# MilchRatchet/Luminary

Hardware: AMD Instinct MI355X
Metric: Mrays/s at 1920x1080, 8 bounces (higher is better)
Workload: dtype f32

## Files before the change

### luminary_amd/csrc/device/dev_scene.h

```cpp
#pragma once

#include <hip/hip_vector_types.h>
#include <stdint.h>

namespace lum {

struct alignas(128) Bvh4Node {
  float lo_x[4], lo_y[4], lo_z[4];
  float hi_x[4], hi_y[4], hi_z[4];
  uint32_t child[4];
  uint32_t pad[4];
};
static_assert(sizeof(Bvh4Node) == 128, "BVH4 node must be one cache line");

#ifndef LUM_BVH8
#define LUM_BVH8 0
#endif
struct alignas(128) Bvh8Node {
  float origin[3];
  uint8_t exp[3], pad0;
  uint32_t child[8];
  uint8_t lo_x[8], lo_y[8], lo_z[8], hi_x[8], hi_y[8], hi_z[8];
  uint32_t pad[8];
};
// ... 127 lines not shown
#endif
  const uint2* sobol_table;
  uint32_t sobol_first, sobol_count, sobol_stride;
};

struct PathQueue {
  float4* origin_t;
  float4* dir_slot;
  uint4* aux;
  uint4* hit_id;
  uint32_t* hit_scene_tri;
  uint32_t* parent;
};
constexpr uint32_t kParentDeferred = 0x80000000u, kParentMask = 0x7FFFFFFFu;

struct NeeQueue {
  float4* geo_color_light;
  float4* bsdf_ray_prob;
  float4* bsdf_weight_sum;
  uint4* ambient;
  uint4* sun;
  uint32_t* amb_path;
  float4* sun_water;
  float4* amb_t1;
  float4* amb_t2;
};

struct ShadowQueue {
  float4* origin_dist;
  float4* dir_out;
  uint4* ids;
  float4* vis;
  uint32_t* light_items;
  uint32_t capacity;
};

struct FusedResolve {
  PathQueue prev;
  NeeQueue nee_prev;
  ShadowQueue fallback;
  uint32_t* ended;
  const uint32_t* ended_prev;
};

constexpr uint32_t kVolumeShadowKinds = 19, kVolumeKindSun = 15, kVolumeKindAmbient = 16, kVolumeKindSun2 = 17, kVolumeKindAmbient2 = 18;
constexpr uint32_t kShadowKindAmbient2 = 4, kShadowKindSun2 = 5, kSurfaceShadowKindsWater = 6;
struct CloudQueue {
  uint32_t* items;
  float4* result;
  float* hit_dist;
  uint32_t capacity;
};
struct VolumeQueue {
  float4* bridge;
  uint4* sky;
  float4* weight;
  float4* sun_water;
  float4* amb_t1;
  float4* amb_t2;
  uint32_t* items;
};

struct PassParams {
  const uint32_t* pixels;
  uint32_t num_pixels, batch, first_sample;
};
// ... 58 lines not shown
```

### luminary_amd/csrc/device/kernels.h

```cpp
#pragma once

#include "kernel_shadow.h"
#include "dev_sky.h"
#include "dev_volume.h"
#include "dev_particle.h"
#include "dev_water.h"
#include "dev_cloud_march.h"

LUM_NS_BEGIN

constexpr int kBlock = 256;
#ifndef LUM_SHADE_WAVES
#define LUM_SHADE_WAVES 3
#endif
#ifndef LUM_CLOUD_WAVES
#define LUM_CLOUD_WAVES 4
#endif
#ifndef LUM_CLOUD_PERSISTENT
#define LUM_CLOUD_PERSISTENT 1
#endif
#ifndef LUM_HIT_COMPACT
#define LUM_HIT_COMPACT 1
#endif
#ifndef LUM_FEATURE_WAVES
// ... 167 lines not shown
  if (mat.roughness_tex != kTextureNone) roughness = texture_load(sc, mat.roughness_tex, tex_coords, true, make_float4(0.5f, 0.0f, 0.0f, 0.0f)).x;
  if (mat.flags & kDMatRoughnessAsSmoothness) roughness = 1.0f - roughness;
  roughness = fmaxf(roughness, 2e-2f);
  if ((state & kStDeltaPath) == 0) roughness = fmaxf(roughness, mat.roughness_clamp);
  uint32_t flags = mat.flags & kDMatSubstrateMask;
  if (mat.metallic_tex == kTextureNone && (mat.flags & kDMatMetallic)) flags |= kMatMetallic;
  if (mat.flags & kDMatColoredTransparency) flags |= kMatColoredTransparency;
  if (inside) flags |= kMatRefractionInside;
  const float other_ior = medium_ior_peek(medium, inside);
  const float ior_in = inside ? mat.refraction_index : other_ior;
  const float ior_out = inside ? other_ior : mat.refraction_index;
  if (((flags & kMatSubstrateMask) == kMatTranslucent) && (fabsf(1.0f - ior_in / ior_out) < 1e-4f)) {
    if ((flags & kMatColoredTransparency) == 0) albedo = col(lerpf(1.0f, albedo.r, alpha), lerpf(1.0f, albedo.g, alpha), lerpf(1.0f, albedo.b, alpha));
    alpha = 0.0f;
    flags |= kMatColoredTransparency;
  }
  GeoContext g;
  g.instance_id = inst; g.tri_id = tri;
  g.normal = xf_rot(tf, normal);
  g.face_normal_packed = normal_pack(face);
  g.position = position;
  g.V = ray_world * -1.0f;
  g.state = state;
  g.params.flags = flags;
  g.params.set(albedo, alpha, roughness, emission, ior_in / ior_out);
  return g;
}

LUM_DEV void add_to_result(float4* results, uint32_t slot, Col v) {
  if (!any_positive(v)) return;
  float4 r = results[slot];
  r.x += v.r; r.y += v.g; r.z += v.b;
  results[slot] = r;
}

struct ResolveRecords { uint4 aux; uint32_t slot; float4 cl, lc; uint4 amb; };
LUM_DEV ResolveRecords load_resolve_records(const PathQueue& in, const NeeQueue& nee, uint32_t i) {
  ResolveRecords r;
  r.aux = ld_stream(&in.aux[i]);
  r.slot = fbits(reinterpret_cast<const float*>(&in.dir_slot[i])[3]);
  r.cl = ld_stream(&nee.geo_color_light[i]);
  r.lc = ld_stream(&nee.bsdf_weight_sum[i]);
  r.amb = ld_stream(&nee.ambient[i]);
  return r;
}
template <int kAmbient>
LUM_DEV bool resolve_records(const DeviceScene& sc, const PathQueue& in, const NeeQueue& nee, const ShadowQueue& sq, float4* results, uint32_t i, bool lights_present, float ambient_vis,
                             const ResolveRecords& r, const uint32_t* hit_word = nullptr) {
  const uint4 aux = r.aux;
  const uint32_t slot = r.slot;
  const bool geo_allowed = lights_present && ((aux.w & kStVolumeScattered) == 0);
  const float4 cl = r.cl, lc = r.lc;
  const uint4 amb = r.amb;
  const bool deferred = kAmbient == 2 && hit_word != nullptr;
  const bool need_geo = fbits(cl.w) != kLightIdInvalid && geo_allowed, need_bsdf = lc.w != 0.0f, need_amb = kAmbient != 1 && !deferred && (amb.x != 0 || amb.y != 0);
  const float4 zero = make_float4(0.0f, 0.0f, 0.0f, 0.0f);
  float4 vg = zero, vb = zero, va = zero;
  uint32_t word = 0u;
  if (deferred) word = *hit_word;
  if (need_geo) vg = ld_stream(&sq.vis[i]);
  if (need_bsdf) vb = ld_stream(&sq.vis[sq.capacity + i]);
  if (need_amb) va = ld_stream(&sq.vis[2u * sq.capacity + i]);
  const float4 before = results[slot];
  if (deferred) {
    if (!(word & kHitTriHit)) { if (word & kHitTriCutout) return false; ambient_vis = 1.0f; }
    else { if ((word & (kHitTriBeyondEps | kHitTriOpaque)) != (kHitTriBeyondEps | kHitTriOpaque)) return false; ambient_vis = 0.0f; }
// ... 361 lines not shown
        LUM_LAP(clock, 4);
        if (kSkyMode != kSkyConstantColor) {
          uint4 sun = make_uint4(0u, 0u, 0u, 0u);
          Col sun_light; V3 sun_dir;
          bool have_sun;
          if (kWater && top_volume == kVolumeOcean) have_sun = sun_caustic_sample(sc, sky_view(sc), g, smp, 0u, top_volume, second_volume, sun_light, sun_dir);
          else {
            have_sun = sample_sun(sc, sky_view(sc), lf, g, smp, sun_light, sun_dir);
            if (have_sun && top_volume != kVolumeNone) sun_light = sun_light * volume_transmittance(sc, top_volume, g.position, sun_dir, kFltMax);
          }
          if (have_sun) {
            const U2 c = record_pack(sun_light), r = ray_pack(sun_dir);
            sun = make_uint4(c.x, c.y, r.x, r.y);
            if (c.x != 0 || c.y != 0) {
              want_sun = true;
              const V3 ar = ray_unpack(r);
              s_sun_dir = make_float4(ar.x, ar.y, ar.z, kFltMax);
              if (kWater) {
                const SkyRayPlan plan = plan_sun_ray(sc, hit_origin, hid.x, top_volume, true, ar);
                s_sun_dir.w = plan.limit;
                nee.sun_water[i] = make_float4(plan.fresnel_factor, 0.0f, 0.0f, bitsf(sky_ray_flags(plan)));
                if (plan.second && !plan.total_reflection) {
                  want_sun2 = true;
                  s_sun2_o = make_float4(plan.second_origin.x, plan.second_origin.y, plan.second_origin.z, kFltMax);
                  s_sun2_d = make_float4(plan.second_dir.x, plan.second_dir.y, plan.second_dir.z, 0.0f);
                }
              }
            }
          }
          st_stream(&nee.sun[i], sun);
          LUM_LAP(clock, 5);
        }
        if (kStage == 0) st_stream(&nee.geo_color_light[i], geo_cl);
        st_stream(&nee.bsdf_ray_prob[i], bs_rp); st_stream(&nee.bsdf_weight_sum[i], bs_ws);
        st_stream(&nee.ambient[i], amb);

        const float roughness = g.params.roughness();
        bool is_delta;
        if (bounce.transparent_pass) {
          const float ior = g.params.ior();
          const float rs = (ior >= 1.0f) ? ior : 1.0f / ior;
          is_delta = roughness * fminf(rs - 1.0f, 1.0f) <= 0.05f;
        }
        else is_delta = bounce.microfacet_based && (roughness <= 0.05f);
        const bool pass_through = is_pass_through(g, bounce);

        Col record = record_in;
        const Col emission = g.params.emission();
        if (any_positive(emission)) add_to_result(results, slot, emission * record);
        record = record * bounce.weight;

        uint32_t new_state = state | kStUseIgnoreHandle;
        if (kSkyMode != kSkyDefault && !pass_through) new_state &= ~kStAllowAmbient; else new_state |= kStAllowAmbient;
        if (!is_delta) new_state &= ~kStDeltaPath;
        if (!pass_through) new_state &= ~(kStCameraDirection | kStAllowEmission);

        survive = true;
        if ((state & kStDeltaPath) == 0) {
          const float value = importance(record);
          if (value < sc.cam_rr_threshold) {
            const float p = (value > 0.0f) ? fmaxf(value / sc.cam_rr_threshold, 1.0f / 8.0f) : 0.0f;
            if (smp.next1(kRndRussianRoulette) > p) survive = false;
            else record = record * (1.0f / p);
          }
        }
        if (survive) {
          uint32_t medium = aux.z;
// ... 1 lines not shown
            const bool inside = (g.params.flags & kMatRefractionInside) != 0;
            float new_ior = 1.0f;
            if (!inside) new_ior = medium_ior_peek(medium, inside) / g.params.ior();
            medium = medium_ior_modify(medium, new_ior, !inside);
          }
          const U2 rp = record_pack(record);
          n_o = make_float4(g.position.x, g.position.y, g.position.z, kFltMax);
          n_d = make_float4(bounce.ray.x, bounce.ray.y, bounce.ray.z, d4.w);
          n_aux = make_uint4(rp.x, rp.y, medium, new_state);
          n_hid = make_uint4(g.instance_id, g.tri_id, hid.z, hid.w);
        }
        }
      }
    }
    if (kStage == 1) {
      const unsigned long long bg = __ballot(want_geo);
      if (bg) {
        uint32_t base = 0;
        if (lane == (uint32_t) __builtin_ctzll(bg)) base = atomicAdd(ctrl + kCtlShadowItems, (uint32_t) __popcll(bg));
        base = __shfl(base, __builtin_ctzll(bg));
        if (want_geo) {
          const uint32_t j = base + (uint32_t) __popcll(bg & below);
          st_stream(&sq.origin_dist[j], make_float4(s_origin.x, s_origin.y, s_origin.z, s_geo_dir.w));
          st_stream(&sq.dir_out[j], make_float4(s_geo_dir.x, s_geo_dir.y, s_geo_dir.z, bitsf(i)));
          st_stream(&sq.ids[j], s_geo_ids);
        }
      }
      continue;
    }
    const bool amb_deferred = reuse_ambient && want_amb && survive;
    if (amb_deferred) { want_amb = false; vertices += 1u << 16; }
    LUM_LAP(clock, 6);
    const unsigned long long ballot = __ballot(survive);
    const unsigned long long bg = __ballot(want_geo), ba = __ballot(want_amb), bn = __ballot(want_sun), bl = __ballot(want_lq);
    const unsigned long long b2a = kWater ? __ballot(want_amb2) : 0ull, b2s = kWater ? __ballot(want_sun2) : 0ull;
    const uint32_t ng = (uint32_t) __popcll(bg), na = (uint32_t) __popcll(ba), ns = (uint32_t) __popcll(bn), na2 = (uint32_t) __popcll(b2a);
    const unsigned long long be = announce_children ? __ballot(valid && !survive) : 0ull;
    const uint32_t want_count = (lane == 0) ? (uint32_t) __popcll(ballot) : (lane == 1) ? ng + na + ns + na2 + (uint32_t) __popcll(b2s) : (lane == 2) ? (uint32_t) __popcll(bl) :
                                (lane == 3) ? (uint32_t) __popcll(be) : 0u;
    uint32_t* const want_word = (lane == 0) ? count_out : (lane == 1) ? ctrl + kCtlShadowItems : (lane == 2) ? ctrl + kCtlLightItems : ctrl + kCtlSkyItems;
    uint32_t reserved = 0;
    if (want_count) reserved = atomicAdd(want_word, want_count);
    const uint32_t base_out = __builtin_amdgcn_readlane(reserved, 0), base_shadow = __builtin_amdgcn_readlane(reserved, 1), base_light = __builtin_amdgcn_readlane(reserved, 2);
    uint32_t amb_path = kNoAmbientPath;
    if (survive) {
      const uint32_t j = base_out + (uint32_t) __popcll(ballot & below);
      st_stream(&out.origin_t[j], n_o); st_stream(&out.dir_slot[j], n_d); st_stream(&out.aux[j], n_aux); st_stream(&out.hit_id[j], n_hid);
      amb_path = amb_deferred ? j : kNoAmbientPath;
      if (announce_children) out.parent[j] = i | (amb_deferred ? kParentDeferred : 0u);
    }
    if (reuse_ambient && valid && !announce_children) nee.amb_path[i] = amb_path;
    if (be != 0ull && valid && !survive) fused_dev->ended[__builtin_amdgcn_readlane(reserved, 3) + (uint32_t) __popcll(be & below)] = i;
    if (want_geo) {
      const uint32_t j = base_shadow + (uint32_t) __popcll(bg & below);
      st_stream(&sq.origin_dist[j], make_float4(s_origin.x, s_origin.y, s_origin.z, s_geo_dir.w));
      st_stream(&sq.dir_out[j], make_float4(s_geo_dir.x, s_geo_dir.y, s_geo_dir.z, bitsf(i)));
      st_stream(&sq.ids[j], s_geo_ids);
    }
    if (want_amb) {
      const uint32_t j = base_shadow + ng + (uint32_t) __popcll(ba & below);
      st_stream(&sq.origin_dist[j], make_float4(s_origin.x, s_origin.y, s_origin.z, s_amb_dir.w));
      st_stream(&sq.dir_out[j], make_float4(s_amb_dir.x, s_amb_dir.y, s_amb_dir.z, bitsf(2u * sq.capacity + i)));
      st_stream(&sq.ids[j], make_uint4(0xFFFFFFFFu, 0u, s_geo_ids.z, s_geo_ids.w));
    }
    if (want_sun) {
      const uint32_t j = base_shadow + ng + na + (uint32_t) __popcll(bn & below);
      st_stream(&sq.origin_dist[j], make_float4(s_origin.x, s_origin.y, s_origin.z, s_sun_dir.w));
      st_stream(&sq.dir_out[j], make_float4(s_sun_dir.x, s_sun_dir.y, s_sun_dir.z, bitsf(3u * sq.capacity + i)));
      st_stream(&sq.ids[j], make_uint4(0xFFFFFFFFu, 0u, s_geo_ids.z, s_geo_ids.w));
    }
    if (kWater) {
      if (want_amb2) {
        const uint32_t j = base_shadow + ng + na + ns + (uint32_t) __popcll(b2a & below);
        sq.origin_dist[j] = s_amb2_o;
        sq.dir_out[j] = make_float4(s_amb2_d.x, s_amb2_d.y, s_amb2_d.z, bitsf(kShadowKindAmbient2 * sq.capacity + i));
        sq.ids[j] = make_uint4(0xFFFFFFFFu, 0u, 0xFFFFFFFFu, 0u);
      }
      if (want_sun2) {
        const uint32_t j = base_shadow + ng + na + ns + na2 + (uint32_t) __popcll(b2s & below);
        sq.origin_dist[j] = s_sun2_o;
        sq.dir_out[j] = make_float4(s_sun2_d.x, s_sun2_d.y, s_sun2_d.z, bitsf(kShadowKindSun2 * sq.capacity + i));
        sq.ids[j] = make_uint4(0xFFFFFFFFu, 0u, 0xFFFFFFFFu, 0u);
      }
    }
    if (want_lq) sq.light_items[base_light + (uint32_t) __popcll(bl & below)] = i;
    LUM_LAP(clock, 7);
  }
  clock.flush();
  uint32_t deferred = vertices >> 16;
  vertices &= 0xFFFFu;
#pragma unroll
  for (int off = 32; off > 0; off >>= 1) { vertices += __shfl_down(vertices, off); deferred += __shfl_down(deferred, off); }
  if ((threadIdx.x & 63) == 0 && vertices) atomicAdd((unsigned long long*) &counters[kCntVertices], (unsigned long long) vertices);
  if ((threadIdx.x & 63) == 0 && deferred) atomicAdd((unsigned long long*) &counters[kCntAmbientDeferred], (unsigned long long) deferred);
}

__global__ __launch_bounds__(kBlock) void k_shade_debug(DeviceScene sc, PathQueue in, float4* results, const uint32_t* ctrl) {
  const uint32_t n = ctrl[kCtlPaths];
  for (uint32_t i = blockIdx.x * kBlock + threadIdx.x; i < n; i += gridDim.x * kBlock) {
    const float4 o4 = in.origin_t[i], d4 = in.dir_slot[i];
    const uint4 aux = in.aux[i], hid = in.hit_id[i];
    const V3 origin = v3(o4.x, o4.y, o4.z), ray = v3(d4.x, d4.y, d4.z);
    Col result = splat(0.0f);
    if (hid.x == kHitSky) {
      if (sc.shading_mode == 1u) {
        if (sc.sky_mode == kSkyDefault) {
          if (sc.sky_lut_transmittance && sc.sky_lut_multiscattering) {
            const SkyView sky = sky_view(sc);
            const Sampler smp{sc.bluenoise_2d, hid.z & 0xFFFFu, hid.z >> 16, path_sample_id(hid.w), 0u};
            result = sky_get_color(sc, sky, world_to_sky(sky, origin), ray, kFltMax, true, (int) sky.steps, smp.next1(kRndSkyStepOffset));
          }
        }
        else if (sc.sky_mode == kSkyHdri) result = sky_hdri_color(sc, origin, ray, kStCameraDirection);
        else result = col(sc.sky_constant_color[0], sc.sky_constant_color[1], sc.sky_constant_color[2]);
      }
      else if (sc.shading_mode == 4u) result = col(0.0f, 0.63f, 1.0f);
    }
    else if (hid.x == kHitOcean) {
// ... 51 lines not shown

__global__ __launch_bounds__(kBlock, LUM_FEATURE_WAVES) void k_sky_inscattering(DeviceScene sc, PathQueue in, float4* results, const uint32_t* ctrl, uint32_t depth_const) {
  const uint32_t n = ctrl[kCtlPaths];
  const SkyView sky = sky_view(sc);
  for (uint32_t i = blockIdx.x * kBlock + threadIdx.x; i < n; i += gridDim.x * kBlock) {
    const uint4 hid = in.hit_id[i];
    if (hid.x == kHitSky) continue;
    const float4 o4 = in.origin_t[i], d4 = in.dir_slot[i];
    uint4 aux = in.aux[i];
    const Sampler smp{sc.bluenoise_2d, hid.z & 0xFFFFu, hid.z >> 16, path_sample_id(hid.w), depth_const};
    Col record = record_unpack(U2{aux.x, aux.y});
    const Col c = sky_trace_inscattering(sc, sky, world_to_sky(sky, v3(o4.x, o4.y, o4.z)), v3(d4.x, d4.y, d4.z), o4.w * 0.001f, record, depth_const == 0u,
                                         smp.next1(kRndSkyInscatteringStep), smp.next1(kRndSkyStepOffset));
    add_to_result(results, fbits(d4.w), c);
    const U2 rp = record_pack(record);
    aux.x = rp.x; aux.y = rp.y;
    in.aux[i] = aux;
  }
}

__global__ __launch_bounds__(kBlock) void k_light_query(DeviceScene sc, PathQueue in, NeeQueue nee, ShadowQueue sq, uint32_t* ctrl, uint32_t depth_const,
                                                        uint64_t* counters) {
  const uint32_t n = ctrl[kCtlLightItems];
  const uint32_t lane = threadIdx.x & 63;
  const unsigned long long below = (1ull << lane) - 1ull;
  RayStats st{0, 0, 0};
  uint32_t light_queries = 0;
  const uint32_t rounds = (n + gridDim.x * kBlock - 1) / (gridDim.x * kBlock);
  for (uint32_t round = 0; round < rounds; round++) {
    const uint32_t item = (round * gridDim.x + blockIdx.x) * kBlock + threadIdx.x;
    bool want = false;
    float4 s_origin, s_dir; uint4 s_ids; uint32_t i = 0;
    if (item < n) {
      i = sq.light_items[item];
      const uint4 hid = in.hit_id[i];
      const float4 o4 = in.origin_t[i], d4 = in.dir_slot[i];
      const V3 hit_origin = v3(o4.x, o4.y, o4.z) + v3(d4.x, d4.y, d4.z) * o4.w;
      const float4 rp = nee.bsdf_ray_prob[i], ws = nee.bsdf_weight_sum[i];
      const V3 ray = v3(rp.x, rp.y, rp.z);
      const Sampler smp{sc.bluenoise_2d, hid.z & 0xFFFFu, hid.z >> 16, path_sample_id(hid.w), depth_const};
      uint32_t num_hits = 0;
      const uint32_t light_id = light_query(sc, hit_origin, ray, hid.x, hid.y, smp.next1(kRndLightBsdfTrace), num_hits, st);
      light_queries++;
      bool valid = light_id != kLightIdInvalid;
      float dist = kFltMax;
      uint2 handle = make_uint2(0xFFFFFFFFu, 0u);
      Col lc = splat(0.0f);
      if (light_id != kLightIdInvalid) {
        handle = sc.light_tri_handles[light_id];
        const TableLight entry = load_tri_light_table(sc, light_id);
        const TriLight& tl = entry.tri;
        F2 uv;
        dist = intersect_triangle(tl.vertex, tl.edge1, tl.edge2, hit_origin, ray, uv);
        if (dist != kFltMax) {
          lc = entry.textured ? tri_light_color(sc, tl, uv) : entry.color;
          const float mis = (ws.w == 0.0f) ? 1.0f : mis_base(rp.w, tri_light_solid_angle(tl, hit_origin), importance(lc) * entry.area, dist * dist, ws.w);
          lc = lc * (mis * num_hits);
          lc = lc * col(ws.x, ws.y, ws.z);
        }
        else valid = false;
      }
      nee.bsdf_weight_sum[i] = make_float4(lc.r, lc.g, lc.b, valid ? 1.0f : 0.0f);
      if (valid && (sc.fog_active || sc.ocean_active)) {
        const Col seen = volume_transmittance(sc, sc.ocean_active ? volume_stack_peek(hid.w, false) : (uint32_t) kVolumeFog, hit_origin, ray, dist);
        nee.bsdf_ray_prob[i] = make_float4(seen.r, seen.g, seen.b, 0.0f);
      }
      if (valid) {
        want = true;
        s_origin = make_float4(hit_origin.x, hit_origin.y, hit_origin.z, dist);
        s_dir = make_float4(ray.x, ray.y, ray.z, bitsf(sq.capacity + i));
        s_ids = make_uint4(handle.x, handle.y, hid.x, hid.y);
      }
    }
    const unsigned long long bw = __ballot(want);
    if (bw) {
      uint32_t base = 0;
      if (lane == 0) base = atomicAdd(ctrl + kCtlShadowItems, (uint32_t) __popcll(bw));
      base = __builtin_amdgcn_readfirstlane(base);
      if (want) {
        const uint32_t j = base + (uint32_t) __popcll(bw & below);
        sq.origin_dist[j] = s_origin; sq.dir_out[j] = s_dir; sq.ids[j] = s_ids;
      }
    }
  }
#pragma unroll
  for (int off = 32; off > 0; off >>= 1) light_queries += __shfl_down(light_queries, off);
  if ((threadIdx.x & 63) == 0 && light_queries) atomicAdd((unsigned long long*) &counters[kCntLightBvh], (unsigned long long) light_queries);
  flush_stats(counters, st, 0, kCntLightBvh, kCntNodesLight, kCntTrisLight);
}

LUM_DEV bool resolves_here(uint32_t hit_type) {
  return !(hit_type > kHitTriangleLimit && !particle_is_hit(hit_type) && hit_type != kHitOcean);
}

__global__ __launch_bounds__(kBlock) void k_resolve(DeviceScene sc, PathQueue in, NeeQueue nee, ShadowQueue sq, float4* results, const uint32_t* ctrl) {
  const uint32_t n = ctrl[kCtlPaths];
  const bool lights_present = sc.light_tree_root != nullptr && sc.num_lights > 0;
  for (uint32_t i = blockIdx.x * kBlock + threadIdx.x; i < n; i += gridDim.x * kBlock) {
    if (!resolves_here(in.hit_id[i].x)) continue;
    resolve_vertex<false>(sc, in, nee, sq, results, i, lights_present, 0.0f);
  }
}

__global__ __launch_bounds__(kBlock) void k_resolve_ended(DeviceScene sc, PathQueue in, NeeQueue nee, ShadowQueue sq, float4* results, const uint32_t* ctrl, const uint32_t* list) {
// ... 233 lines not shown
              }
            }
          }
        }
      }
      const float random_choice = smp.next1(kRndBsdfGiResampling);
      const F2 random_dir = smp.next2(kRndBsdfGiDiffuse);
      const V3 bounce = je_phase_sample(sc.particles_phase, ray, random_dir, random_choice);
      uint4 amb = make_uint4(0u, 0u, 0u, 0u);
      if (sc.sky_mode != kSkyDefault) {
        const U2 c = record_pack(sky_color_no_compute(sc, position, bounce, 0u) * albedo), r = ray_pack(bounce);
        amb = make_uint4(c.x, c.y, r.x, r.y);
        if (c.x != 0 || c.y != 0) {
          const V3 ar = ray_unpack(r);
          if (sc.ocean_active) {
            const SkyRayPlan plan = plan_ambient_ray(sc, position, hid.x, top_volume, second_volume, true, ar);
            if (!plan.valid) amb = make_uint4(0u, 0u, r.x, r.y);
            else {
              want_amb = true;
              s_amb_dir = make_float4(ar.x, ar.y, ar.z, plan.limit);
              nee.amb_t1[i] = make_float4(plan.t1.r, plan.t1.g, plan.t1.b, plan.fresnel_factor);
              nee.amb_t2[i] = make_float4(plan.t2.r, plan.t2.g, plan.t2.b, bitsf(sky_ray_flags(plan)));
              if (plan.second && !plan.total_reflection) {
                want_amb2 = true;
                s_amb2_o = make_float4(plan.second_origin.x, plan.second_origin.y, plan.second_origin.z, kFltMax);
                s_amb2_d = make_float4(plan.second_dir.x, plan.second_dir.y, plan.second_dir.z, 0.0f);
              }
            }
          }
          else { want_amb = true; s_amb_dir = make_float4(ar.x, ar.y, ar.z, kFltMax); }
        }
      }
      nee.geo_color_light[i] = geo_cl;
      nee.bsdf_ray_prob[i] = make_float4(0.0f, 0.0f, 1.0f, 0.0f);
      nee.bsdf_weight_sum[i] = make_float4(0.0f, 0.0f, 0.0f, 0.0f);
      nee.ambient[i] = amb;
      if (sc.sky_mode != kSkyConstantColor) nee.sun[i] = sun;
      uint32_t new_state = state & ~(kStDeltaPath | kStCameraDirection | kStAllowEmission | kStUseIgnoreHandle);
      if (sc.sky_mode != kSkyDefault) new_state &= ~kStAllowAmbient; else new_state |= kStAllowAmbient;
      Col record = record_unpack(U2{aux.x, aux.y}) * albedo;
      survive = true;
      if ((state & kStDeltaPath) == 0) {
        const float value = importance(record);
        if (value < sc.cam_rr_threshold) {
          const float p = (value > 0.0f) ? fmaxf(value / sc.cam_rr_threshold, 1.0f / 8.0f) : 0.0f;
          if (smp.next1(kRndRussianRoulette) > p) survive = false;
          else record = record * (1.0f / p);
        }
      }
      if (survive) {
        const U2 rp = record_pack(record);
        n_o = make_float4(position.x, position.y, position.z, kFltMax);
        n_d = make_float4(bounce.x, bounce.y, bounce.z, d4.w);
        n_aux = make_uint4(rp.x, rp.y, aux.z, new_state);
        n_hid = make_uint4(0u, 0u, hid.z, hid.w);
      }
    }
    const unsigned long long ballot = __ballot(survive);
    if (ballot) {
      uint32_t base = 0;
      if (lane == 0) base = atomicAdd(count_out, (uint32_t) __popcll(ballot));
      base = __builtin_amdgcn_readfirstlane(base);
      if (survive) {
        const uint32_t j = base + (uint32_t) __popcll(ballot & below);
        out.origin_t[j] = n_o; out.dir_slot[j] = n_d; out.aux[j] = n_aux; out.hit_id[j] = n_hid;
      }
    }
// ... 95 lines not shown
      const float4 o4 = in.origin_t[i], d4 = in.dir_slot[i];
      const uint4 aux = in.aux[i], hid = in.hit_id[i];
      const uint32_t state = aux.w;
      const V3 ray = v3(d4.x, d4.y, d4.z);
      const V3 position = v3(o4.x, o4.y, o4.z) + ray * o4.w;
      const Sampler smp{sc.bluenoise_2d, hid.z & 0xFFFFu, hid.z >> 16, path_sample_id(hid.w), depth_const};
      const GeoContext g = ocean_context(sc, position, ray, state, aux.z);
      const uint32_t top_volume = volume_stack_peek(hid.w, false);
      const LocalFrame lf = local_frame(sc, g);
      s_origin = make_float4(position.x, position.y, position.z, 0.0f);
      float4 bs_rp = make_float4(0.0f, 0.0f, 1.0f, 0.0f), bs_ws = make_float4(0.0f, 0.0f, 0.0f, 0.0f);
      if (lights_present && (state & kStVolumeScattered) == 0) {
        const LightDirSample lb = sample_light_direction(lf, g, smp);
        bs_rp = make_float4(lb.ray.x, lb.ray.y, lb.ray.z, lb.probability);
        if (lb.probability != 0.0f) { want_lq = true; bs_ws = make_float4(lb.weight.r, lb.weight.g, lb.weight.b, 0.0f); }
      }
      uint4 sun = make_uint4(0u, 0u, 0u, 0u);
      if (sun_allowed) {
        Col sun_light; V3 sun_dir;
        if (sample_sun(sc, sky_view(sc), lf, g, smp, sun_light, sun_dir)) {
          sun_light = sun_light * volume_transmittance(sc, top_volume, g.position, sun_dir, kFltMax);
          const U2 c = record_pack(sun_light), r = ray_pack(sun_dir);
          sun = make_uint4(c.x, c.y, r.x, r.y);
          if (c.x != 0 || c.y != 0) {
            want_sun = true;
            const V3 ar = ray_unpack(r);
            s_sun_dir = make_float4(ar.x, ar.y, ar.z, kFltMax);
            nee.sun_water[i] = make_float4(1.0f, 0.0f, 0.0f, bitsf(0u));
          }
        }
      }
      const BounceSample bounce = sample_bounce(lf, g, smp, 0);
      nee.geo_color_light[i] = make_float4(0.0f, 0.0f, 0.0f, bitsf(kLightIdInvalid));
      nee.bsdf_ray_prob[i] = bs_rp; nee.bsdf_weight_sum[i] = bs_ws;
      nee.ambient[i] = make_uint4(0u, 0u, 0u, 0u);
      if (sc.sky_mode != kSkyConstantColor) nee.sun[i] = sun;
      Col record = record_unpack(U2{aux.x, aux.y}) * bounce.weight;
      const float shift_length = 8.0f * kEps * (1.0f + sc.ocean_amplitude) * (1.0f + fabsf(sc.ocean_height));
      const V3 bounce_pos = g.position + g.normal * (bounce.transparent_pass ? -shift_length : shift_length);
      const uint32_t new_state = state & ~(kStCameraDirection | kStAllowEmission | kStUseIgnoreHandle);
      survive = true;
      if ((state & kStDeltaPath) == 0) {
        const float value = importance(record);
        if (value < sc.cam_rr_threshold) {
          const float p = (value > 0.0f) ? fmaxf(value / sc.cam_rr_threshold, 1.0f / 8.0f) : 0.0f;
          if (smp.next1(kRndRussianRoulette) > p) survive = false;
          else record = record * (1.0f / p);
        }
      }
      if (survive) {
        uint32_t medium = aux.z, volumes = hid.w;
        if (bounce.transparent_pass) {
          const bool inside = (g.params.flags & kMatRefractionInside) != 0;
          medium = medium_ior_modify(medium, sc.ocean_refractive_index, !inside);
          volumes = volume_stack_modify(volumes, kVolumeOcean, !inside);
        }
        const U2 rp = record_pack(record);
        n_o = make_float4(bounce_pos.x, bounce_pos.y, bounce_pos.z, kFltMax);
        n_d = make_float4(bounce.ray.x, bounce.ray.y, bounce.ray.z, d4.w);
        n_aux = make_uint4(rp.x, rp.y, medium, new_state);
        n_hid = make_uint4(0u, 0u, hid.z, volumes);
      }
    }
    const unsigned long long ballot = __ballot(survive);
    if (ballot) {
      uint32_t base = 0;
      if (lane == 0) base = atomicAdd(count_out, (uint32_t) __popcll(ballot));
      base = __builtin_amdgcn_readfirstlane(base);
      if (survive) {
        const uint32_t j = base + (uint32_t) __popcll(ballot & below);
        out.origin_t[j] = n_o; out.dir_slot[j] = n_d; out.aux[j] = n_aux; out.hit_id[j] = n_hid;
      }
    }
    const unsigned long long bn = __ballot(want_sun);
    if (bn) {
      uint32_t base = 0;
      if (lane == 0) base = atomicAdd(ctrl + kCtlShadowItems, (uint32_t) __popcll(bn));
      base = __builtin_amdgcn_readfirstlane(base);
      if (want_sun) {
        const uint32_t j = base + (uint32_t) __popcll(bn & below);
        sq.origin_dist[j] = make_float4(s_origin.x, s_origin.y, s_origin.z, s_sun_dir.w);
        sq.dir_out[j] = make_float4(s_sun_dir.x, s_sun_dir.y, s_sun_dir.z, bitsf(3u * sq.capacity + i));
        sq.ids[j] = make_uint4(0xFFFFFFFFu, 0u, kHitOcean, 0u);
      }
    }
    const unsigned long long bl = __ballot(want_lq);
    if (bl) {
      uint32_t base = 0;
      if (lane == 0) base = atomicAdd(ctrl + kCtlLightItems, (uint32_t) __popcll(bl));
      base = __builtin_amdgcn_readfirstlane(base);
      if (want_lq) sq.light_items[base + (uint32_t) __popcll(bl & below)] = i;
    }
  }
}

__global__ __launch_bounds__(kBlock) void k_clouds_list(DeviceScene sc, PathQueue in, CloudQueue cq, uint32_t* ctrl) {
  const uint32_t n = ctrl[kCtlPaths];
  const SkyView sky = sky_view(sc);
  const uint32_t lane = threadIdx.x & 63;
  const unsigned long long below = (1ull << lane) - 1ull;
  const uint32_t rounds = (n + gridDim.x * kBlock - 1) / (gridDim.x * kBlock);
  constexpr uint32_t kListRounds = 8;
  uint32_t masks = 0;
  for (uint32_t round = 0; round < rounds; round++) {
    const uint32_t i = (round * gridDim.x + blockIdx.x) * kBlock + threadIdx.x;
    uint32_t mask = 0;
    if (i < n && in.hit_id[i].x != kHitInvalid) {
      const float4 o4 = in.origin_t[i], d4 = in.dir_slot[i];
      const V3 sky_origin = world_to_sky(sky, v3(o4.x, o4.y, o4.z)), ray = v3(d4.x, d4.y, d4.z);
      const float limit = o4.w * 0.001f;
#pragma unroll
      for (int l = 0; l < 3; l++) if (cloud_layer_intersection(sc, sky_origin, ray, limit, l).x != kFltMax) mask |= 1u << l;
    }
    const uint32_t slot = round % kListRounds;
    masks |= mask << (3u * slot);
    if (slot + 1u == kListRounds || round + 1u == rounds) {
      uint32_t total = 0;
#pragma unroll
      for (uint32_t b = 0; b < 3u * kListRounds; b++) total += (uint32_t) __popcll(__ballot((masks >> b) & 1u));
      if (total) {
        uint32_t base = 0;
        if (lane == 0) base = atomicAdd(ctrl + kCtlCloudItems, total);
        base = __builtin_amdgcn_readfirstlane(base);
        const uint32_t group_start = round - slot;
// ... 655 lines not shown
```

### luminary_amd/csrc/host/core.hip

```cpp
#include <hip/hip_runtime.h>

#include <algorithm>
#include <chrono>
#include <cfloat>
#include <queue>
#include <cstdio>
#include <cstdlib>
#include <cstring>
#include <map>
#include <memory>
#include <mutex>
#include <string>
#include <thread>
#include <tuple>
#include <vector>

#include "../../../include/lum_core.h"
#include "../device/kernels.h"
#include "../device/dev_output.h"
#include "../device/dev_adaptive.h"
#include "../device/wavefront_table_impl.h"
#include <hipcub/hipcub.hpp>
#include <rccl/rccl.h>
#include "bvh_build.h"
// ... 222 lines not shown
void free_adaptive(LumContext* ctx) {
  LumContext::Adaptive& a = ctx->adaptive;
  void* bufs[] = {a.d_stage_counts, a.d_block_tasks, a.d_block_task_end, a.d_block_variance, a.d_partial, a.d_scan_temp, a.d_block_mask};
  for (void* b : bufs) if (b) (void) hipFree(b);
  a = LumContext::Adaptive();
}

void free_work(LumContext* ctx) {
  if (ctx->work_block) (void) hipFree(ctx->work_block);
  ctx->work_block = nullptr;
  if (ctx->fused_block) (void) hipFree(ctx->fused_block);
  ctx->fused_block = nullptr; ctx->fused_capacity = 0; ctx->d_fused = nullptr;
  ctx->fused_refused_capacity = 0;
  ctx->queue[2] = PathQueue{}; ctx->nee2 = NeeQueue{}; ctx->fallback = ShadowQueue{};
  for (int k = 0; k < 3; k++) ctx->queue[k].parent = nullptr;
  ctx->capacity = 0;
  ctx->work_shadow_kinds = 0;
  ctx->cloud = CloudQueue{};
  for (int k = 0; k < 4; k++) { if (ctx->sort_planes[k]) (void) hipFree(ctx->sort_planes[k]); ctx->sort_planes[k] = nullptr; }
  ctx->sort_queue = PathQueue{}; ctx->sort_queue_capacity = 0;
  if (ctx->d_sobol) (void) hipFree(ctx->d_sobol);
  ctx->d_sobol = nullptr; ctx->sobol_entries = 0;
}

int ensure_work(LumContext* ctx, uint32_t paths) {
  const bool volumes = ctx->scene.fog_active || ctx->scene.ocean_active;
  const uint32_t kinds = volumes ? kVolumeShadowKinds : 4u;
  const bool clouds = ctx->scene.cloud_active && ctx->scene.sky_mode == kSkyDefault;
  if (clouds && paths >= (1u << 30)) { ctx->error = "pass too large for the cloud march list (2^30 paths)"; return 1; }
  if (paths <= ctx->capacity && kinds <= ctx->work_shadow_kinds && (!clouds || ctx->cloud.items)) return 0;
  if (paths < ctx->capacity) paths = ctx->capacity;
  free_work(ctx);
  const size_t n = paths;
  const size_t bytes = n * (2 * 68 + 84 + 16 + (size_t) kinds * 64 + 4 + (kinds > 4u ? 100 + 48 : 0) + (clouds ? 3 * (4 + 16 + 4) : 0)) + 56 * 256;
  HIP_TRY(ctx, hipMalloc(&ctx->work_block, bytes));
  char* p = (char*) ctx->work_block;
  auto take = [&](size_t sz) { char* r = p; p += (sz + 255) & ~(size_t) 255; return r; };
  for (int k = 0; k < 2; k++) {
    ctx->queue[k].origin_t = (float4*) take(n * 16);
    ctx->queue[k].dir_slot = (float4*) take(n * 16);
    ctx->queue[k].aux      = (uint4*) take(n * 16);
    ctx->queue[k].hit_id   = (uint4*) take(n * 16);
    ctx->queue[k].hit_scene_tri = (uint32_t*) take(n * 4);
  }
  ctx->nee.geo_color_light = (float4*) take(n * 16);
  ctx->nee.bsdf_ray_prob   = (float4*) take(n * 16);
  ctx->nee.bsdf_weight_sum = (float4*) take(n * 16);
  ctx->nee.ambient         = (uint4*) take(n * 16);
  ctx->nee.sun             = (uint4*) take(n * 16);
  ctx->nee.amb_path        = (uint32_t*) take(n * 4);
  ctx->d_results           = (float4*) take(n * 16);
  ctx->shadow.origin_dist  = (float4*) take(kinds * n * 16);
  ctx->shadow.dir_out      = (float4*) take(kinds * n * 16);
  ctx->shadow.ids          = (uint4*) take(kinds * n * 16);
  ctx->shadow.vis          = (float4*) take(kinds * n * 16);
  ctx->shadow.light_items  = (uint32_t*) take(n * 4);
  ctx->shadow.capacity     = paths;
  ctx->volume = VolumeQueue{};
  ctx->nee.sun_water = nullptr; ctx->nee.amb_t1 = nullptr; ctx->nee.amb_t2 = nullptr;
  if (kinds > 4u) {
    ctx->volume.bridge = (float4*) take(n * 16);
    ctx->volume.sky    = (uint4*) take(n * 16);
    ctx->volume.weight = (float4*) take(n * 16);
    ctx->volume.sun_water = (float4*) take(n * 16);
    ctx->volume.amb_t1 = (float4*) take(n * 16);
    ctx->volume.amb_t2 = (float4*) take(n * 16);
    ctx->volume.items  = (uint32_t*) take(n * 4);
    ctx->nee.sun_water = (float4*) take(n * 16);
    ctx->nee.amb_t1    = (float4*) take(n * 16);
    ctx->nee.amb_t2    = (float4*) take(n * 16);
  }
  ctx->cloud = CloudQueue{};
  if (clouds) {
    ctx->cloud.items    = (uint32_t*) take(3 * n * 4);
    ctx->cloud.result   = (float4*) take(3 * n * 16);
    ctx->cloud.hit_dist = (float*) take(3 * n * 4);
    ctx->cloud.capacity = paths;
  }
  ctx->work_shadow_kinds = kinds;
  ctx->capacity = paths;
  return 0;
}

int upload_fused_records(LumContext* ctx, hipStream_t stream) {
  FusedResolve by_depth[6];
  for (int d = 0; d < 6; d++) {
    by_depth[d].prev = ctx->queue[(d + 2) % 3];
    by_depth[d].nee_prev = (d & 1) ? ctx->nee : ctx->nee2;
    by_depth[d].fallback = ctx->fallback;
// ... 2723 lines not shown
```

Measured before the change: 3822.

## Pack light-query inputs into compacted SoA records instead of gathering by path index

Shading kernels now reserve light-query slots at the point where the BSDF ray is produced and write a compacted 64-byte record holding hit origin, ray, weight sum, probability and id words. The light-query kernel reads these contiguous records directly instead of indirecting through light_items and gathering origin_t, dir_slot, hit_id and the NEE buffers by path index. This is meant to replace scattered gathers with coalesced streaming loads. In exchange it adds 64 bytes per path of work memory, an extra wave-level atomic at the store site, and changes which NEE fields are written for paths that do not queue a light query.

```diff
diff --git a/luminary_amd/csrc/device/dev_scene.h b/luminary_amd/csrc/device/dev_scene.h
--- a/luminary_amd/csrc/device/dev_scene.h
+++ b/luminary_amd/csrc/device/dev_scene.h
@@ -183,6 +183,7 @@
   uint4* ids;
   float4* vis;
   uint32_t* light_items;
+  uint4* light_records;
   uint32_t capacity;
 };
 
diff --git a/luminary_amd/csrc/device/kernels.h b/luminary_amd/csrc/device/kernels.h
--- a/luminary_amd/csrc/device/kernels.h
+++ b/luminary_amd/csrc/device/kernels.h
@@ -223,6 +223,26 @@
   float4 r = results[slot];
   r.x += v.r; r.y += v.g; r.z += v.b;
   results[slot] = r;
+}
+
+struct LightRecord { V3 hit_origin, ray; float4 weight_sum; float probability; uint32_t self_inst, self_tri, pixel, sample_word, path; };
+LUM_DEV void light_record_store(const ShadowQueue& sq, uint32_t q, V3 hit_origin, V3 ray, float4 weight_sum, float probability, uint4 hid, uint32_t path) {
+  const size_t c = sq.capacity;
+  st_stream(&sq.light_records[q], make_uint4(fbits(hit_origin.x), fbits(hit_origin.y), fbits(hit_origin.z), hid.x));
+  st_stream(&sq.light_records[c + q], make_uint4(fbits(ray.x), fbits(ray.y), fbits(ray.z), hid.y));
+  st_stream(&sq.light_records[2u * c + q], make_uint4(fbits(weight_sum.x), fbits(weight_sum.y), fbits(weight_sum.z), fbits(weight_sum.w)));
+  st_stream(&sq.light_records[3u * c + q], make_uint4(fbits(probability), hid.z, hid.w, path));
+}
+LUM_DEV LightRecord light_record_load(const ShadowQueue& sq, uint32_t q) {
+  const size_t c = sq.capacity;
+  const uint4 w0 = ld_stream(&sq.light_records[q]), w1 = ld_stream(&sq.light_records[c + q]), w2 = ld_stream(&sq.light_records[2u * c + q]),
+              w3 = ld_stream(&sq.light_records[3u * c + q]);
+  LightRecord r;
+  r.hit_origin = v3(bitsf(w0.x), bitsf(w0.y), bitsf(w0.z)); r.self_inst = w0.w;
+  r.ray = v3(bitsf(w1.x), bitsf(w1.y), bitsf(w1.z)); r.self_tri = w1.w;
+  r.weight_sum = make_float4(bitsf(w2.x), bitsf(w2.y), bitsf(w2.z), bitsf(w2.w));
+  r.probability = bitsf(w3.x); r.pixel = w3.y; r.sample_word = w3.z; r.path = w3.w;
+  return r;
 }
 
 struct ResolveRecords { uint4 aux; uint32_t slot; float4 cl, lc; uint4 amb; };
@@ -650,7 +670,16 @@
           LUM_LAP(clock, 5);
         }
         if (kStage == 0) st_stream(&nee.geo_color_light[i], geo_cl);
-        st_stream(&nee.bsdf_ray_prob[i], bs_rp); st_stream(&nee.bsdf_weight_sum[i], bs_ws);
+        {
+          const unsigned long long bl = __ballot(want_lq);
+          if (bl) {
+            uint32_t base = 0;
+            if (lane == (uint32_t) __builtin_ctzll(bl)) base = atomicAdd(ctrl + kCtlLightItems, (uint32_t) __popcll(bl));
+            base = __shfl(base, __builtin_ctzll(bl));
+            if (want_lq) light_record_store(sq, base + (uint32_t) __popcll(bl & below), hit_origin, v3(bs_rp.x, bs_rp.y, bs_rp.z), bs_ws, bs_rp.w, hid, i);
+          }
+          if (!want_lq) st_stream(&nee.bsdf_weight_sum[i], bs_ws);
+        }
         st_stream(&nee.ambient[i], amb);
 
         const float roughness = g.params.roughness();
@@ -718,16 +747,15 @@
     if (amb_deferred) { want_amb = false; vertices += 1u << 16; }
     LUM_LAP(clock, 6);
     const unsigned long long ballot = __ballot(survive);
-    const unsigned long long bg = __ballot(want_geo), ba = __ballot(want_amb), bn = __ballot(want_sun), bl = __ballot(want_lq);
+    const unsigned long long bg = __ballot(want_geo), ba = __ballot(want_amb), bn = __ballot(want_sun);
     const unsigned long long b2a = kWater ? __ballot(want_amb2) : 0ull, b2s = kWater ? __ballot(want_sun2) : 0ull;
     const uint32_t ng = (uint32_t) __popcll(bg), na = (uint32_t) __popcll(ba), ns = (uint32_t) __popcll(bn), na2 = (uint32_t) __popcll(b2a);
     const unsigned long long be = announce_children ? __ballot(valid && !survive) : 0ull;
-    const uint32_t want_count = (lane == 0) ? (uint32_t) __popcll(ballot) : (lane == 1) ? ng + na + ns + na2 + (uint32_t) __popcll(b2s) : (lane == 2) ? (uint32_t) __popcll(bl) :
-                                (lane == 3) ? (uint32_t) __popcll(be) : 0u;
-    uint32_t* const want_word = (lane == 0) ? count_out : (lane == 1) ? ctrl + kCtlShadowItems : (lane == 2) ? ctrl + kCtlLightItems : ctrl + kCtlSkyItems;
+    const uint32_t want_count = (lane == 0) ? (uint32_t) __popcll(ballot) : (lane == 1) ? ng + na + ns + na2 + (uint32_t) __popcll(b2s) : (lane == 2) ? (uint32_t) __popcll(be) : 0u;
+    uint32_t* const want_word = (lane == 0) ? count_out : (lane == 1) ? ctrl + kCtlShadowItems : ctrl + kCtlSkyItems;
     uint32_t reserved = 0;
     if (want_count) reserved = atomicAdd(want_word, want_count);
-    const uint32_t base_out = __builtin_amdgcn_readlane(reserved, 0), base_shadow = __builtin_amdgcn_readlane(reserved, 1), base_light = __builtin_amdgcn_readlane(reserved, 2);
+    const uint32_t base_out = __builtin_amdgcn_readlane(reserved, 0), base_shadow = __builtin_amdgcn_readlane(reserved, 1);
     uint32_t amb_path = kNoAmbientPath;
     if (survive) {
       const uint32_t j = base_out + (uint32_t) __popcll(ballot & below);
@@ -736,7 +764,7 @@
       if (announce_children) out.parent[j] = i | (amb_deferred ? kParentDeferred : 0u);
     }
     if (reuse_ambient && valid && !announce_children) nee.amb_path[i] = amb_path;
-    if (be != 0ull && valid && !survive) fused_dev->ended[__builtin_amdgcn_readlane(reserved, 3) + (uint32_t) __popcll(be & below)] = i;
+    if (be != 0ull && valid && !survive) fused_dev->ended[__builtin_amdgcn_readlane(reserved, 2) + (uint32_t) __popcll(be & below)] = i;
     if (want_geo) {
       const uint32_t j = base_shadow + (uint32_t) __popcll(bg & below);
       st_stream(&sq.origin_dist[j], make_float4(s_origin.x, s_origin.y, s_origin.z, s_geo_dir.w));
@@ -769,7 +797,6 @@
         sq.ids[j] = make_uint4(0xFFFFFFFFu, 0u, 0xFFFFFFFFu, 0u);
       }
     }
-    if (want_lq) sq.light_items[base_light + (uint32_t) __popcll(bl & below)] = i;
     LUM_LAP(clock, 7);
   }
   clock.flush();
@@ -887,15 +914,13 @@
     bool want = false;
     float4 s_origin, s_dir; uint4 s_ids; uint32_t i = 0;
     if (item < n) {
-      i = sq.light_items[item];
-      const uint4 hid = in.hit_id[i];
-      const float4 o4 = in.origin_t[i], d4 = in.dir_slot[i];
-      const V3 hit_origin = v3(o4.x, o4.y, o4.z) + v3(d4.x, d4.y, d4.z) * o4.w;
-      const float4 rp = nee.bsdf_ray_prob[i], ws = nee.bsdf_weight_sum[i];
-      const V3 ray = v3(rp.x, rp.y, rp.z);
-      const Sampler smp{sc.bluenoise_2d, hid.z & 0xFFFFu, hid.z >> 16, path_sample_id(hid.w), depth_const};
+      const LightRecord rec = light_record_load(sq, item);
+      i = rec.path;
+      const V3 hit_origin = rec.hit_origin, ray = rec.ray;
+      const float4 ws = rec.weight_sum;
+      const Sampler smp{sc.bluenoise_2d, rec.pixel & 0xFFFFu, rec.pixel >> 16, path_sample_id(rec.sample_word), depth_const};
       uint32_t num_hits = 0;
-      const uint32_t light_id = light_query(sc, hit_origin, ray, hid.x, hid.y, smp.next1(kRndLightBsdfTrace), num_hits, st);
+      const uint32_t light_id = light_query(sc, hit_origin, ray, rec.self_inst, rec.self_tri, smp.next1(kRndLightBsdfTrace), num_hits, st);
       light_queries++;
       bool valid = light_id != kLightIdInvalid;
       float dist = kFltMax;
@@ -909,7 +934,7 @@
         dist = intersect_triangle(tl.vertex, tl.edge1, tl.edge2, hit_origin, ray, uv);
         if (dist != kFltMax) {
           lc = entry.textured ? tri_light_color(sc, tl, uv) : entry.color;
-          const float mis = (ws.w == 0.0f) ? 1.0f : mis_base(rp.w, tri_light_solid_angle(tl, hit_origin), importance(lc) * entry.area, dist * dist, ws.w);
+          const float mis = (ws.w == 0.0f) ? 1.0f : mis_base(rec.probability, tri_light_solid_angle(tl, hit_origin), importance(lc) * entry.area, dist * dist, ws.w);
           lc = lc * (mis * num_hits);
           lc = lc * col(ws.x, ws.y, ws.z);
         }
@@ -917,14 +942,14 @@
       }
       nee.bsdf_weight_sum[i] = make_float4(lc.r, lc.g, lc.b, valid ? 1.0f : 0.0f);
       if (valid && (sc.fog_active || sc.ocean_active)) {
-        const Col seen = volume_transmittance(sc, sc.ocean_active ? volume_stack_peek(hid.w, false) : (uint32_t) kVolumeFog, hit_origin, ray, dist);
+        const Col seen = volume_transmittance(sc, sc.ocean_active ? volume_stack_peek(rec.sample_word, false) : (uint32_t) kVolumeFog, hit_origin, ray, dist);
         nee.bsdf_ray_prob[i] = make_float4(seen.r, seen.g, seen.b, 0.0f);
       }
       if (valid) {
         want = true;
         s_origin = make_float4(hit_origin.x, hit_origin.y, hit_origin.z, dist);
         s_dir = make_float4(ray.x, ray.y, ray.z, bitsf(sq.capacity + i));
-        s_ids = make_uint4(handle.x, handle.y, hid.x, hid.y);
+        s_ids = make_uint4(handle.x, handle.y, rec.self_inst, rec.self_tri);
       }
     }
     const unsigned long long bw = __ballot(want);
@@ -1224,7 +1249,6 @@
         }
       }
       nee.geo_color_light[i] = geo_cl;
-      nee.bsdf_ray_prob[i] = make_float4(0.0f, 0.0f, 1.0f, 0.0f);
       nee.bsdf_weight_sum[i] = make_float4(0.0f, 0.0f, 0.0f, 0.0f);
       nee.ambient[i] = amb;
       if (sc.sky_mode != kSkyConstantColor) nee.sun[i] = sun;
@@ -1386,7 +1410,16 @@
       }
       const BounceSample bounce = sample_bounce(lf, g, smp, 0);
       nee.geo_color_light[i] = make_float4(0.0f, 0.0f, 0.0f, bitsf(kLightIdInvalid));
-      nee.bsdf_ray_prob[i] = bs_rp; nee.bsdf_weight_sum[i] = bs_ws;
+      {
+        const unsigned long long bl = __ballot(want_lq);
+        if (bl) {
+          uint32_t base = 0;
+          if (lane == (uint32_t) __builtin_ctzll(bl)) base = atomicAdd(ctrl + kCtlLightItems, (uint32_t) __popcll(bl));
+          base = __shfl(base, __builtin_ctzll(bl));
+          if (want_lq) light_record_store(sq, base + (uint32_t) __popcll(bl & below), position, v3(bs_rp.x, bs_rp.y, bs_rp.z), bs_ws, bs_rp.w, hid, i);
+        }
+        if (!want_lq) nee.bsdf_weight_sum[i] = bs_ws;
+      }
       nee.ambient[i] = make_uint4(0u, 0u, 0u, 0u);
       if (sc.sky_mode != kSkyConstantColor) nee.sun[i] = sun;
       Col record = record_unpack(U2{aux.x, aux.y}) * bounce.weight;
@@ -1437,13 +1470,6 @@
         sq.dir_out[j] = make_float4(s_sun_dir.x, s_sun_dir.y, s_sun_dir.z, bitsf(3u * sq.capacity + i));
         sq.ids[j] = make_uint4(0xFFFFFFFFu, 0u, kHitOcean, 0u);
       }
-    }
-    const unsigned long long bl = __ballot(want_lq);
-    if (bl) {
-      uint32_t base = 0;
-      if (lane == 0) base = atomicAdd(ctrl + kCtlLightItems, (uint32_t) __popcll(bl));
-      base = __builtin_amdgcn_readfirstlane(base);
-      if (want_lq) sq.light_items[base + (uint32_t) __popcll(bl & below)] = i;
     }
   }
 }
diff --git a/luminary_amd/csrc/host/core.hip b/luminary_amd/csrc/host/core.hip
--- a/luminary_amd/csrc/host/core.hip
+++ b/luminary_amd/csrc/host/core.hip
@@ -278,7 +278,7 @@
   if (paths < ctx->capacity) paths = ctx->capacity;
   free_work(ctx);
   const size_t n = paths;
-  const size_t bytes = n * (2 * 68 + 84 + 16 + (size_t) kinds * 64 + 4 + (kinds > 4u ? 100 + 48 : 0) + (clouds ? 3 * (4 + 16 + 4) : 0)) + 56 * 256;
+  const size_t bytes = n * (2 * 68 + 84 + 16 + (size_t) kinds * 64 + 4 + 64 + (kinds > 4u ? 100 + 48 : 0) + (clouds ? 3 * (4 + 16 + 4) : 0)) + 57 * 256;
   HIP_TRY(ctx, hipMalloc(&ctx->work_block, bytes));
   char* p = (char*) ctx->work_block;
   auto take = [&](size_t sz) { char* r = p; p += (sz + 255) & ~(size_t) 255; return r; };
@@ -301,6 +301,7 @@
   ctx->shadow.ids          = (uint4*) take(kinds * n * 16);
   ctx->shadow.vis          = (float4*) take(kinds * n * 16);
   ctx->shadow.light_items  = (uint32_t*) take(n * 4);
+  ctx->shadow.light_records = (uint4*) take(4 * n * 16);
   ctx->shadow.capacity     = paths;
   ctx->volume = VolumeQueue{};
   ctx->nee.sun_water = nullptr; ctx->nee.amb_t1 = nullptr; ctx->nee.amb_t2 = nullptr;
```

Measured after the change: 3525 (median of 2 runs). -7.8%, worse.
